# simonsobs/Pixell.jl

Measured on AMD Instinct MI355X. Metric: Mpix/s CAR bilinear reproject (Float64) + % HBM roofline, 1/2/4/8 MI355X, higher is better.
Workload: dtype f64

## Files before the change

pixell.jl_amd/csrc/pxl_kernels.hip:

```cpp
#include <hip/hip_runtime.h>

#include <algorithm>
#include <mutex>
#include <vector>
#include <cmath>
#include <cstdarg>
#include <cstdio>
#include <cstring>
#include <new>
#include <type_traits>

#include "pxl_device.h"

using namespace pxl;

static thread_local char g_err[512] = "";

static int fail(int code, const char* fmt, ...) {
    va_list ap;
    va_start(ap, fmt);
    vsnprintf(g_err, sizeof(g_err), fmt, ap);
    va_end(ap);
    return code;
}
// ... 387 lines not shown
                                    "this library can see is one it loaded itself (%s): a foreign communicator belongs to another instance", nc.where);
        int nranks = 0, me = -1;
        if (nc.CommCount((ncclComm_t)comm, &nranks) != ncclSuccess || nc.CommUserRank((ncclComm_t)comm, &me) != ncclSuccess)
            return fail(PXL_EINVAL, "sharded_step: not a usable RCCL communicator");
        for (int pass = 0; pass < 2; ++pass) {
            const pxl_halo_xfer* x = pass == 0 ? sends : recvs;
            for (int i = 0; i < (pass == 0 ? nsends : nrecvs); ++i) {
                if (x[i].peer < 0 || x[i].peer >= nranks) return fail(PXL_EINVAL, "sharded_step: peer %d outside the communicator (%d ranks)", x[i].peer, nranks);
                if (x[i].nrows < 1 || x[i].row0 < lo || x[i].row0 + x[i].nrows > hi) return fail(PXL_EINVAL, "sharded_step: transfer rows outside the plan's source window");
                if (pass == 0 && (x[i].row0 < own_row0 || x[i].row0 + x[i].nrows > own_row0 + own_nrows))
                    return fail(PXL_EINVAL, "sharded_step: a rank can only send rows it owns");
            }
        }
        if (!pl->comm_stream) {
            HIP_TRY(hipStreamCreateWithFlags(&pl->comm_stream, hipStreamNonBlocking));
            HIP_TRY(hipEventCreateWithFlags(&pl->ev_ready, hipEventDisableTiming));
            HIP_TRY(hipEventCreateWithFlags(&pl->ev_halo, hipEventDisableTiming));
        }
        HIP_TRY(hipEventRecord(pl->ev_ready, st));
        HIP_TRY(hipStreamWaitEvent(pl->comm_stream, pl->ev_ready, 0));
        const size_t esz = sizeof(T);
        const ncclDataType_t dt = std::is_same<T, float>::value ? ncclFloat32 : ncclFloat64;
        ncclResult_t r = nc.GroupStart();
        for (int i = 0; i < nsends && r == ncclSuccess; ++i)
            for (int64_t c = 0; c < pl->nc && r == ncclSuccess; ++c)
                r = nc.Send((const char*)src + ((c * pl->src_nrows + (sends[i].row0 - lo)) * pl->nx) * esz,
                            (size_t)(sends[i].nrows * pl->nx), dt, sends[i].peer, (ncclComm_t)comm, pl->comm_stream);
        for (int i = 0; i < nrecvs && r == ncclSuccess; ++i)
            for (int64_t c = 0; c < pl->nc && r == ncclSuccess; ++c)
                r = nc.Recv((char*)src + ((c * pl->src_nrows + (recvs[i].row0 - lo)) * pl->nx) * esz,
                            (size_t)(recvs[i].nrows * pl->nx), dt, recvs[i].peer, (ncclComm_t)comm, pl->comm_stream);
        const ncclResult_t rend = nc.GroupEnd();
        if (r == ncclSuccess) r = rend;
        if (r != ncclSuccess) return fail(PXL_EHIP, "sharded_step: RCCL send/recv failed: %s", nc.GetErrorString(r));
        HIP_TRY(hipEventRecord(pl->ev_halo, pl->comm_stream));
    }
    rc = pxl_reproject_build_tables(pl, stream);
    if (rc) return rc;
    int64_t i_lo = 0, i_hi = pl->dst_nrows;
    if (exchange) {
        if (pl->cov_have_lo != own_row0 || pl->cov_have_hi != own_row0 + own_nrows || pl->cov_hi < pl->cov_lo) {
            rc = pxl_reproject_plan_rows_covered(pl, own_row0, own_row0 + own_nrows, &pl->cov_lo, &pl->cov_hi);
            if (rc) return rc;
            pl->cov_have_lo = own_row0; pl->cov_have_hi = own_row0 + own_nrows;
        }
        i_lo = pl->cov_lo; i_hi = pl->cov_hi;
    }
    if (i_hi > i_lo) {
        rc = reproject_rows_impl<T>(pl, src, dst, i_lo, i_hi - i_lo, stream);
        if (rc) return rc;
    }
    if (exchange) {
        HIP_TRY(hipStreamWaitEvent(st, pl->ev_halo, 0));
        if (i_hi > i_lo) {
            if (i_lo > 0) { rc = reproject_rows_impl<T>(pl, src, dst, 0, i_lo, stream); if (rc) return rc; }
            if (i_hi < pl->dst_nrows) rc = reproject_rows_impl<T>(pl, src, dst, i_hi, pl->dst_nrows - i_hi, stream);
        } else {
            rc = reproject_rows_impl<T>(pl, src, dst, 0, pl->dst_nrows, stream);
        }
    }
    return rc;
}

static unsigned int* last_exact_word(int64_t total_tiles = -1, int64_t* total_out = nullptr) {
    DeviceState* d = device_state();
    if (!d) return nullptr;
    std::lock_guard<std::mutex> lock(g_dev_mu);
    if (!d->last_exact) {
        if (hipMalloc((void**)&d->last_exact, 64) != hipSuccess || hipMemset(d->last_exact, 0, 64) != hipSuccess) {
            (void)hipGetLastError(); d->last_exact = nullptr; return nullptr;
        }
    }
    if (total_tiles >= 0) d->generic_tiles = total_tiles;
    if (total_out) *total_out = d->generic_tiles;
    return d->last_exact;
}

static int generic_params(const char* who, const pxl_car_wcs* wcs_in, int proj_in, const int64_t* shape_in,
                          const pxl_car_wcs* wcs_out, int proj_out, const int64_t* shape_out, GenericParams* out) {
    if (!wcs_ok(wcs_in) || !wcs_ok(wcs_out)) return fail(PXL_EINVAL, "%s: invalid WCS", who);
    if (!shape_in || !shape_out) return fail(PXL_EINVAL, "%s: null shape", who);
    if (shape_in[0] < 1 || shape_in[1] < 1 || shape_out[0] < 1 || shape_out[1] < 1)
        return fail(PXL_EINVAL, "%s: shapes must be positive", who);
    if ((proj_in != PXL_PROJ_CAR && proj_in != PXL_PROJ_TAN) || (proj_out != PXL_PROJ_CAR && proj_out != PXL_PROJ_TAN))
        return fail(PXL_EINVAL, "%s: unknown projection code", who);
    GenericParams p;
    memset(&p, 0, sizeof(p));
    p.nx = shape_in[0]; p.ny = shape_in[1]; p.nc = 1;
    p.nxo = shape_out[0]; p.nyo = shape_out[1];
    p.proj_in = proj_in; p.proj_out = proj_out;
    p.periodic = (proj_in == PXL_PROJ_CAR) && car_periodic(wcs_in, p.nx);
    if (proj_out == PXL_PROJ_TAN) p.out_tan = tan_setup(*wcs_out); else p.out_car = car_affine(*wcs_out);
    if (proj_in == PXL_PROJ_TAN) p.in_tan = tan_setup(*wcs_in);
    else p.in_car = sky2pix_setup(*wcs_in, p.nx, p.ny, 1, PXL_FORM_DIV);
    *out = p;
    return PXL_OK;
}

struct LatticeWs { double2* lat; int32_t* flag; unsigned int* counter; size_t bytes; };
static LatticeWs lattice_layout(void* mem, int64_t ntiles) {
    const size_t lat_bytes = (size_t)ntiles * (PXL_TNX * PXL_TNY) * sizeof(double2), flag_bytes = ((size_t)ntiles * 4 + 15) & ~(size_t)15;
    const uintptr_t b = (uintptr_t)mem;
    return {(double2*)b, (int32_t*)(b + lat_bytes), (unsigned int*)(b + lat_bytes + flag_bytes), lat_bytes + flag_bytes + 16};
}
static hipError_t lattice_build(const GenericParams& p, int64_t gx, int64_t ntiles, const LatticeWs& ws, hipStream_t st) {
    hipError_t e = hipMemsetAsync(ws.counter, 0, 16, st);
    if (e == hipSuccess) hipLaunchKernelGGL(k_generic_lattice, dim3((unsigned)((ntiles + 3) / 4)), dim3(256), 0, st, p, gx, ntiles, ws.lat, ws.flag);
    return e;
}

static int check_sample(const char* who, const pxl_car_wcs* wcs_in, const int64_t shape_in[3], int64_t src_row0, int64_t src_nrows,
                        int64_t n, const double* sky, const void* out, bool no_data) {
    if (!wcs_ok(wcs_in) || !shape_in) return fail(PXL_EINVAL, "%s: invalid WCS/shape", who);
    if (shape_in[0] < 1 || shape_in[1] < 1 || shape_in[2] < 1) return fail(PXL_EINVAL, "%s: shapes must be positive", who);
    if (src_row0 < 0 || src_nrows < 0 || src_row0 + src_nrows > shape_in[1])
        return fail(PXL_EINVAL, "%s: source window outside the map", who);
    if (n < 0 || (n > 0 && (!sky || !out || no_data))) return fail(PXL_EINVAL, "%s: null buffer or negative n", who);
    if (((uintptr_t)sky & 15) != 0) return fail(PXL_EINVAL, "%s: 2xN buffer must be 16-byte aligned", who);
    return PXL_OK;
}

template <class T>
static int sample_impl(const pxl_car_wcs* wcs_in, const int64_t shape_in[3], const T* src, int64_t src_row0,
                       int64_t src_nrows, int64_t n, const double* sky, T* out, void* stream) {
    if (int rc = check_sample("sample", wcs_in, shape_in, src_row0, src_nrows, n, sky, out, !src && src_nrows > 0)) return rc;
    if (n == 0) return PXL_OK;
    Sky2Pix s = sky2pix_setup(*wcs_in, shape_in[0], shape_in[1], 1, PXL_FORM_RECIP);
    dim3 grid(stream_grid((n + PXL_SUNR - 1) / PXL_SUNR, 256));
    hipLaunchKernelGGL((k_sample_bilinear<T>), grid, dim3(256), 0, (hipStream_t)stream, s, src, shape_in[0], shape_in[1],
                       (int32_t)shape_in[2], src_row0, src_nrows, car_periodic(wcs_in, shape_in[0]), n, (const double2*)sky, out);
    return check_launch("k_sample_bilinear");
}

static int spline_shape_check(const char* what, const int64_t shape[3]) {
    if (!shape) return fail(PXL_EINVAL, "%s: null shape", what);
    if (shape[0] < 4 || shape[1] < 4) return fail(PXL_EINVAL, "%s: a cubic spline needs nx, ny >= 4 (got %lld x %lld)", what, (long long)shape[0], (long long)shape[1]);
    if (shape[2] < 1 || shape[2] > 65535) return fail(PXL_EINVAL, "%s: 1 to 65535 components", what);
    if (shape[0] > 400000000 || shape[1] > 400000000) return fail(PXL_EINVAL, "%s: axis too long (<= 4e8 pixels)", what);
    return PXL_OK;
}

template <class T>
static int build_pairs_impl(const int64_t shape_in[3], const T* src, int64_t src_nrows, T* pairs, void* stream) {
    if (pxl_sample_pairs_elems(shape_in, src_nrows) < 0) return PXL_EINVAL;
    if (!pairs || (!src && src_nrows > 0)) return fail(PXL_EINVAL, "sample_build_pairs: null buffer");
    if (((uintptr_t)pairs & 63) != 0) return fail(PXL_EINVAL, "sample_build_pairs: pair buffer must be 64-byte aligned");
    if (shape_in[0] > 0x7fffffffLL) return fail(PXL_EINVAL, "sample_build_pairs: more than 2^31 columns");
    if (shape_in[2] > 65535) return fail(PXL_EINVAL, "sample_build_pairs: more than 65535 components");
    const int64_t nx = shape_in[0], tiles = (src_nrows + 1 + PXL_POS_ROWS - 1) / PXL_POS_ROWS;
    if (tiles > 65535) return fail(PXL_EINVAL, "sample_build_pairs: more than %lld rows per call", 65535LL * PXL_POS_ROWS);
    const int64_t pitch = PairGroup<T>::groups(nx) * PairGroup<T>::E;
    const Fronts f = front_split(tiles, 16, 65535);
    dim3 grid((unsigned)((pitch + 255) / 256), (unsigned)(f.per * f.fronts), (unsigned)shape_in[2]);
    hipLaunchKernelGGL((k_build_rowpairs<T>), grid, dim3(256), 0, (hipStream_t)stream, src, nx, src_nrows, (typename Vec2T<T>::type*)pairs, f.fronts);
    return check_launch("k_build_rowpairs");
}

template <class T>
static int sample_pairs_impl(const pxl_car_wcs* wcs_in, const int64_t shape_in[3], const T* pairs, int64_t src_row0,
                             int64_t src_nrows, int64_t n, const double* sky, T* out, void* stream) {
    if (int rc = check_sample("sample_pairs", wcs_in, shape_in, src_row0, src_nrows, n, sky, out, !pairs)) return rc;
    if (((uintptr_t)pairs & 63) != 0) return fail(PXL_EINVAL, "sample_pairs: pair buffer must be 64-byte aligned");
    if (shape_in[0] > 0x7fffffffLL) return fail(PXL_EINVAL, "sample_pairs: more than 2^31 columns");
    if (n == 0) return PXL_OK;
    Sky2Pix s = sky2pix_setup(*wcs_in, shape_in[0], shape_in[1], 1, PXL_FORM_RECIP);
    dim3 grid(stream_grid((n + PairsUnroll<T>::value - 1) / PairsUnroll<T>::value, 256));
    hipLaunchKernelGGL((k_sample_pairs<T>), grid, dim3(256), 0, (hipStream_t)stream, s, (const typename Vec2T<T>::type*)pairs,
                       shape_in[0], shape_in[1], (int32_t)shape_in[2], src_row0, src_nrows, car_periodic(wcs_in, shape_in[0]), n,
                       (const double2*)sky, out);
    return check_launch("k_sample_pairs");
}

extern "C" {

int pxl_version(void) { return PXL_VERSION; }

size_t pxl_last_error(char* buf, size_t n) {
    size_t len = strlen(g_err);
    if (buf && n) {
        size_t m = len < n - 1 ? len : n - 1;
        memcpy(buf, g_err, m);
        buf[m] = 0;
    }
    return len;
}

int pxl_release_scratch(void) {
    DeviceState* d = device_state();
    if (!d) return fail(PXL_ENODEV, "release_scratch: no current device");
    std::lock_guard<std::mutex> lock(g_dev_mu);
    if (d->pool && hipMemPoolTrimTo(d->pool, 0) != hipSuccess) return fail(PXL_EHIP, "release_scratch: hipMemPoolTrimTo failed");
    return PXL_OK;
}

int pxl_mem_probe_pair(void* a, void* b, size_t window_bytes, int reps, float* us, void* stream) {
    if (!a || !b || !us) return fail(PXL_EINVAL, "mem_probe_pair: null argument");
    if (window_bytes < (64u << 20) || (window_bytes & 63) != 0 || (((uintptr_t)a | (uintptr_t)b) & 15) != 0)
        return fail(PXL_EINVAL, "mem_probe_pair: windows of at least 64 MiB, a multiple of 64 bytes, 16-byte aligned");
    if (reps < 1 || reps > 99) return fail(PXL_EINVAL, "mem_probe_pair: 1..99 repetitions");
    hipStream_t st = (hipStream_t)stream;
    hipEvent_t e0, e1;
    HIP_TRY(hipEventCreate(&e0));
    {
        hipError_t ec = hipEventCreate(&e1);
        if (ec != hipSuccess) { (void)hipEventDestroy(e0); return fail(PXL_EHIP, "hipEventCreate(&e1): %s", hipGetErrorString(ec)); }
    }
    std::vector<float> t(reps);
    int rc = PXL_OK;
    for (int r = -1; r < reps && rc == PXL_OK; ++r) {
        hipError_t e = hipEventRecord(e0, st);
        hipLaunchKernelGGL(k_spread_probe, dim3(8 * 256 * 2), dim3(256), 0, st, (char*)a, (char*)b, window_bytes / 4);
        if (e == hipSuccess) e = hipGetLastError();
        if (e == hipSuccess) e = hipEventRecord(e1, st);
        if (e == hipSuccess) e = hipEventSynchronize(e1);
        float ms = 0.f;
        if (e == hipSuccess) e = hipEventElapsedTime(&ms, e0, e1);
        if (e != hipSuccess) rc = fail(PXL_EHIP, "mem_probe_pair: %s", hipGetErrorString(e));
        else if (r >= 0) t[r] = ms * 1000.f;
    }
    (void)hipEventDestroy(e0);
    (void)hipEventDestroy(e1);
    if (rc) return rc;
    std::sort(t.begin(), t.end());
    *us = t[reps / 2];
    return PXL_OK;
}

#include "pxl_place.h"

int pxl_device_count(void) {
    int n = 0;
    hipError_t e = hipGetDeviceCount(&n);
    if (e != hipSuccess) return fail(PXL_ENODEV, "hipGetDeviceCount: %s", hipGetErrorString(e));
    return n;
}

int pxl_pix2sky_car_f64(const pxl_car_wcs* wcs, int64_t n, const double* pix, double* sky, int wrap_mode,
                        void* stream) {
    if (!wcs_ok(wcs)) return fail(PXL_EINVAL, "pix2sky: invalid WCS");
    if (n < 0 || (n > 0 && (!pix || !sky))) return fail(PXL_EINVAL, "pix2sky: null buffer or negative n");
    if (wrap_mode < PXL_WRAP_NONE || wrap_mode > PXL_WRAP_UNWIND) return fail(PXL_EINVAL, "pix2sky: bad wrap_mode %d", wrap_mode);
    if ((((uintptr_t)pix | (uintptr_t)sky) & 15) != 0) return fail(PXL_EINVAL, "pix2sky: 2xN buffers must be 16-byte aligned");
    if (n == 0) return PXL_OK;
    hipStream_t st = (hipStream_t)stream;
    CarAffine c = car_affine(*wcs);
    const int mode = wrap_mode == PXL_WRAP_REWIND ? 1 : (wrap_mode == PXL_WRAP_UNWIND ? 2 : 0);
    if (wrap_mode == PXL_WRAP_NONE) {
        hipLaunchKernelGGL((k_pix2sky_pairs<1>), dim3(stream_grid(n, 256)), dim3(256), 0, st, c, n, (const double2*)pix,
                           (double2*)sky, mode, (const int32_t*)nullptr);
        return check_launch("k_pix2sky_pairs");
    }
    const dim3 pgrid(stream_grid((n + 1) / 2, 256));
    if (wrap_mode != PXL_WRAP_UNWIND) {
        hipLaunchKernelGGL((k_pix2sky_pairs<2>), pgrid, dim3(256), 0, st, c, n, (const double2*)pix, (double2*)sky, mode,
                           (const int32_t*)nullptr);
        return check_launch("k_pix2sky_pairs");
    }
    const uintptr_t pa = (uintptr_t)pix, sa = (uintptr_t)sky, bytes = (uintptr_t)n * 16;
    if (pa != sa && pa < sa + bytes && sa < pa + bytes) return fail(PXL_EINVAL, "pix2sky: pix and sky may alias exactly or not at all");
    auto pre_rewind = [&](const int32_t* gate) {
        hipLaunchKernelGGL((k_pix2sky_pairs<2>), dim3(std::min(pgrid.x, 2048u)), dim3(256), 0, st, c, n, (const double2*)pix, (double2*)sky, 2, gate);
        return check_launch("k_pix2sky_pairs");
    };
    return unwind_ladder<true>(UwSrcPix2{c, (const double2*)pix, PXL_TWOPI_D, 0.0, 1.0 / PXL_TWOPI_D}, (double2*)sky, n, pa == sa, pre_rewind, st);
}

int pxl_rewind_f64(double* a, int64_t n, double period, double ref_angle, void* stream) {
    if (n < 0 || (n > 0 && !a)) return fail(PXL_EINVAL, "rewind: null buffer or negative n");
    if (!(period > 0.0) || !std::isfinite(period) || !std::isfinite(ref_angle)) return fail(PXL_EINVAL, "rewind: period must be positive and finite");
    if (n == 0) return PXL_OK;
    hipLaunchKernelGGL(k_rewind, dim3(stream_grid((n + 3) / 4, 256)), dim3(256), 0, (hipStream_t)stream, n, a, period, ref_angle, 0,
                       (const int32_t*)nullptr);
    return check_launch("k_rewind");
}

int pxl_unwind_f64(double* a, int64_t n, int nrow, double period, double ref_angle, void* stream) {
    if (n < 0 || (n > 0 && !a)) return fail(PXL_EINVAL, "unwind: null buffer or negative n");
    if (nrow != 1 && nrow != 2) return fail(PXL_EINVAL, "unwind: nrow must be 1 (vector) or 2 (2xN batch)");
    if (!(period > 0.0) || !std::isfinite(period) || !std::isfinite(ref_angle)) return fail(PXL_EINVAL, "unwind: period must be positive and finite");
    if (nrow == 2 && ((uintptr_t)a & 15) != 0) return fail(PXL_EINVAL, "unwind: 2xN buffer must be 16-byte aligned");
    if (n == 0) return PXL_OK;
    hipStream_t st = (hipStream_t)stream;
    const dim3 rgrid(stream_grid(((int64_t)nrow * n + 3) / 4, 256));
    auto pre_rewind = [&](const int32_t* gate) {
        hipLaunchKernelGGL(k_rewind, dim3(std::min(rgrid.x, 2048u)), dim3(256), 0, st, (int64_t)nrow * n, a, period, ref_angle, 1, gate);
        return check_launch("k_rewind");
    };
    if (nrow == 2) return unwind_ladder<false>(UwSrcAng2{(const double2*)a, period, ref_angle, 1.0 / period}, (double2*)a, n, true, pre_rewind, st);
    return unwind_ladder<false>(UwSrcAng1{(const double*)a, period, ref_angle, 1.0 / period}, a, n, true, pre_rewind, st);
}

int pxl_pix2sky_car_soa_f64(const pxl_car_wcs* wcs, int64_t n, const double* ipix, const double* jpix,
                            double* ra, double* dec, int safe, void* stream) {
    if (!wcs_ok(wcs)) return fail(PXL_EINVAL, "pix2sky_soa: invalid WCS");
    if (n < 0 || (n > 0 && (!ipix || !jpix || !ra || !dec))) return fail(PXL_EINVAL, "pix2sky_soa: null buffer or negative n");
    if (n == 0) return PXL_OK;
    const int vec = ((((uintptr_t)ipix | (uintptr_t)jpix | (uintptr_t)ra | (uintptr_t)dec) & 15) == 0) ? 1 : 0;
    hipLaunchKernelGGL(k_pix2sky_soa, dim3(stream_grid((n + 1) / 2, 256)), dim3(256), 0, (hipStream_t)stream,
                       car_affine(*wcs), n, ipix, jpix, ra, dec, safe ? 1 : 0, vec);
    return check_launch("k_pix2sky_soa");
}

int pxl_sky2pix_car_f64(const pxl_car_wcs* wcs, const int64_t shape[2], int64_t n, const double* sky,
                        double* pix, int safe, int form, void* stream) {
    if (!wcs_ok(wcs) || !shape) return fail(PXL_EINVAL, "sky2pix: invalid WCS/shape");
    if (n < 0 || (n > 0 && (!pix || !sky))) return fail(PXL_EINVAL, "sky2pix: null buffer or negative n");
    if (form < 0 || form > 2) return fail(PXL_EINVAL, "sky2pix: bad form %d", form);
// ... 668 lines not shown
```

pixell.jl_amd/csrc/pxl_sample.h:

```cpp
#pragma once

struct GenericParams {
    const double* src; double* dst;
    int64_t nx, ny, nxo, nyo;
    int32_t nc, periodic, proj_in, proj_out;
    CarAffine out_car; TanParams out_tan;
    Sky2Pix in_car; TanParams in_tan;
    unsigned int* exact_tiles;
    unsigned int* exact_tiles_last;
};
__device__ inline void generic_coords(const GenericParams& p, double i, double j, double* x, double* y, bool* visible) {
    double ra, dec;
    if (p.proj_out == PXL_PROJ_TAN) tan_pix2sky(p.out_tan, i, j, &ra, &dec);
    else { ra = p2s_ra(p.out_car, i); dec = p2s_dec(p.out_car, j); }
    *visible = true;
    if (p.proj_in == PXL_PROJ_TAN) {
        tan_sky2pix(p.in_tan, ra, dec, x, y);
        *visible = (p.in_tan.sd0 * sin(dec) + cos(dec) * cos(ra - p.in_tan.a0) * p.in_tan.cd0) > 0.0;
    } else { *x = s2p_x(p.in_car, ra); *y = s2p_y(p.in_car, dec); }
}
__device__ inline void generic_store(const GenericParams& p, int64_t t, double x, double y, bool visible) {
    const int64_t total = p.nxo * p.nyo;
    const bool fin = isfinite(x) && isfinite(y);
    int32_t i0, j0; double fx, fy;
// ... 192 lines not shown
#ifndef PXL_T3_G
#define PXL_T3_G 4
#endif

    constexpr int G = PXL_T3_G;
#pragma unroll
    for (int q0 = 0; q0 < NQ; q0 += G) {
        double fx[G], fy[G];
        int64_t off[G];
        bool ok = true;
#pragma unroll
        for (int g = 0; g < G; ++g) {
            const int r = ry + PXL_TROWS * (q0 + g);
            double x, y;
            coords(r, &x, &y);
            const double flx = floor(x), fly = floor(y);
            fx[g] = x - flx; fy[g] = y - fly;
            const int32_t i0 = (int32_t)flx, j0 = (int32_t)fly;
            ok = ok && (uint32_t)(i0 - 1) < nxm1 && (uint32_t)(j0 - 1) < nym1;
            off[g] = small ? (int64_t)((j0 - 1) * nx32 + (i0 - 1)) : (int64_t)(j0 - 1) * p.nx + (i0 - 1);
        }
        const bool inside = tj0 + ry + PXL_TROWS * (q0 + G - 1) < p.nyo;
        if (inside && __all(ok)) {
            for (int c = 0; c < p.nc; ++c) {
                const double* pl = p.src + (int64_t)c * p.nx * p.ny;
                Pair tp[G], bt[G];
#pragma unroll
                for (int g = 0; g < G; ++g) { tp[g] = *reinterpret_cast<const Pair*>(pl + off[g]); bt[g] = *reinterpret_cast<const Pair*>(pl + off[g] + p.nx); }
#pragma unroll
                for (int g = 0; g < G; ++g) {
                    const double top = (1 - fx[g]) * tp[g].a + fx[g] * tp[g].b;
                    const double bot = (1 - fx[g]) * bt[g].a + fx[g] * bt[g].b;
                    __builtin_nontemporal_store((1 - fy[g]) * top + fy[g] * bot, &p.dst[(int64_t)c * total + (tj0 + ry + PXL_TROWS * (q0 + g)) * p.nxo + i]);
                }
            }
        } else {
#pragma unroll
            for (int g = 0; g < G; ++g)
                if (tj0 + ry + PXL_TROWS * (q0 + g) < p.nyo) slow_rows |= 1u << (q0 + g);
        }
    }
#pragma unroll 1
    while (slow_rows) {
        const int q = __builtin_ctz(slow_rows);
        slow_rows &= slow_rows - 1;
        const int r = ry + PXL_TROWS * q;
        double x, y;
        double sx = 0.0, sy = 0.0;
#pragma unroll
        for (int b = 0; b < PXL_TNY; ++b) { const double wy = c_tile_weights.wy[r][b]; sx = __builtin_fma(wy, colx[b], sx); sy = __builtin_fma(wy, coly[b], sy); }
        x = sx; y = sy;
        generic_store(p, (tj0 + r) * p.nxo + i, x, y, true);
    }
}

#ifndef PXL_SUNR
#define PXL_SUNR 4
#endif
__device__ __noinline__ double2 sample_coords_slow(double a, double d, double ia0, double a0, double rda, double px, double cx,
                                                   double rpx, double id0, double d0, double rdd, double py, double cy, double rpy) {
    return make_double2(rewind(ia0 + (a - a0) * rda, px, cx, rpx), rewind(id0 + (d - d0) * rdd, py, cy, rpy));
}
__device__ inline void sample_coords(const Sky2Pix& s, double a, double d, double* x, double* y) {
    if (s.safe && s.form != PXL_FORM_DIV) {
        bool ok0, ok1;
        *x = rewind_try(s.c.ia0 + (a - s.c.a0) * s.rda, s.px, s.cx, s.rpx, &ok0);
        *y = rewind_try(s.c.id0 + (d - s.c.d0) * s.rdd, s.py, s.cy, s.rpy, &ok1);
        if (__builtin_expect(!(ok0 && ok1), 0)) {
            const double2 r = sample_coords_slow(a, d, s.c.ia0, s.c.a0, s.rda, s.px, s.cx, s.rpx, s.c.id0, s.c.d0, s.rdd, s.py, s.cy, s.rpy);
            *x = r.x; *y = r.y;
        }
        return;
    }
    *x = s2p_x(s, a); *y = s2p_y(s, d);
}
template <typename T>
__global__ __launch_bounds__(256) void k_sample_bilinear(Sky2Pix s, const T* __restrict__ src, int64_t nx,
                                                         int64_t ny, int32_t nc, int64_t row0, int64_t nrows,
                                                         int periodic, int64_t n, const double2* __restrict__ sky,
                                                         T* __restrict__ out) {
    const int64_t chunk = (int64_t)blockDim.x * PXL_SUNR;
    const int64_t plane = nx * nrows;
    for (int64_t k0 = (int64_t)blockIdx.x * chunk + threadIdx.x; k0 < n; k0 += (int64_t)gridDim.x * chunk) {
        double2 ad[PXL_SUNR];
#pragma unroll
        for (int u = 0; u < PXL_SUNR; ++u) {
            int64_t k = k0 + u * blockDim.x;
            ad[u] = (k < n) ? sky[k] : make_double2(0.0, 0.0);
        }
        int64_t o00[PXL_SUNR], o10[PXL_SUNR], o01[PXL_SUNR], o11[PXL_SUNR];
        double fx[PXL_SUNR], fy[PXL_SUNR];
        bool fin[PXL_SUNR];
#pragma unroll
        for (int u = 0; u < PXL_SUNR; ++u) {
            double x = s2p_x(s, ad[u].x), y = s2p_y(s, ad[u].y);
            fin[u] = isfinite(x) && isfinite(y);
            int32_t i0, j0;
            split_cell(x, &i0, &fx[u]);
            split_cell(y, &j0, &fy[u]);
            int64_t ia = i0, ib = (int64_t)i0 + 1;
            bool oka = true, okb = true;
            if (periodic) { ia = wrap_col(ia, nx); ib = wrap_col(ib, nx); }
            else { oka = (ia >= 1 && ia <= nx); okb = (ib >= 1 && ib <= nx); }
            int64_t ja = (int64_t)j0 - 1 - row0, jb = ja + 1;
            bool rowa = (j0 >= 1 && j0 <= ny && ja >= 0 && ja < nrows);
            bool rowb = ((int64_t)j0 + 1 >= 1 && (int64_t)j0 + 1 <= ny && jb >= 0 && jb < nrows);
            o00[u] = (rowa && oka) ? ja * nx + (ia - 1) : -1;
            o10[u] = (rowa && okb) ? ja * nx + (ib - 1) : -1;
            o01[u] = (rowb && oka) ? jb * nx + (ia - 1) : -1;
            o11[u] = (rowb && okb) ? jb * nx + (ib - 1) : -1;
        }
        for (int c = 0; c < nc; ++c) {
            const T* pl = src + (int64_t)c * plane;
            double m00[PXL_SUNR], m10[PXL_SUNR], m01[PXL_SUNR], m11[PXL_SUNR];
            struct __attribute__((packed, aligned(sizeof(T)))) TT { T a, b; };
            bool wide[PXL_SUNR];
#pragma unroll
            for (int u = 0; u < PXL_SUNR; ++u) {
                wide[u] = o00[u] >= 0 && o01[u] >= 0 && o10[u] == o00[u] + 1 && o11[u] == o01[u] + 1;
                const TT ra = *(wide[u] ? reinterpret_cast<const TT*>(pl + o00[u]) : reinterpret_cast<const TT*>(sky));
                const TT rb = *(wide[u] ? reinterpret_cast<const TT*>(pl + o01[u]) : reinterpret_cast<const TT*>(sky));
                m00[u] = (double)ra.a; m10[u] = (double)ra.b; m01[u] = (double)rb.a; m11[u] = (double)rb.b;
            }
#pragma unroll
            for (int u = 0; u < PXL_SUNR; ++u) {
                if (__builtin_expect(!wide[u], 0)) {
                    m00[u] = o00[u] >= 0 ? (double)pl[o00[u]] : 0.0;
                    m10[u] = o10[u] >= 0 ? (double)pl[o10[u]] : 0.0;
                    m01[u] = o01[u] >= 0 ? (double)pl[o01[u]] : 0.0;
                    m11[u] = o11[u] >= 0 ? (double)pl[o11[u]] : 0.0;
                }
            }
#pragma unroll
            for (int u = 0; u < PXL_SUNR; ++u) {
                int64_t k = k0 + u * blockDim.x;
                double top = (1 - fx[u]) * m00[u] + fx[u] * m10[u];
                double bot = (1 - fx[u]) * m01[u] + fx[u] * m11[u];
                double v = (1 - fy[u]) * top + fy[u] * bot;
                if (k < n) out[(int64_t)c * n + k] = (T)(fin[u] ? v : __builtin_nan(""));
            }
        }
    }
}

template <typename T> struct Vec2T;
template <> struct Vec2T<double> { typedef double2 type; };
template <> struct Vec2T<float>  { typedef float2 type; };

template <typename T> struct PairGroup {
    static constexpr int E = 64 / (2 * (int)sizeof(T));
    static constexpr int C = E - 1;
    __host__ __device__ static inline int64_t groups(int64_t nx) { return (nx + C - 1) / C; }
};
template <typename T>
__global__ __launch_bounds__(256) void k_build_rowpairs(const T* __restrict__ src, int64_t nx, int64_t nrows,
                                                        typename Vec2T<T>::type* __restrict__ pairs, int fronts) {
    typedef typename Vec2T<T>::type T2;
    constexpr int E = PairGroup<T>::E, C = PairGroup<T>::C;
    const int64_t pitch = PairGroup<T>::groups(nx) * E;
    const int64_t t = (int64_t)blockIdx.x * blockDim.x + threadIdx.x;
    if (t >= pitch) return;
    const int64_t g = t / E, e = t - g * E;
    int64_t i = g * C + e;
    if (i >= nx) i %= nx;
    const int64_t c = blockIdx.z;
    const T* pl = src + c * nx * nrows;
    T2* out = pairs + c * pitch * (nrows + 1);
    const int64_t per = (gridDim.y + fronts - 1) / fronts;
    const int64_t yy = fronts > 1 ? (int64_t)(blockIdx.y % fronts) * per + blockIdx.y / fronts : (int64_t)blockIdx.y;
    const int64_t p0 = yy * PXL_POS_ROWS;
    if (p0 > nrows) return;
    const int64_t p1 = (p0 + PXL_POS_ROWS <= nrows) ? p0 + PXL_POS_ROWS : nrows + 1;
    T above = (p0 >= 1) ? pl[(p0 - 1) * nx + i] : (T)0;
    for (int64_t p = p0; p < p1; ++p) {
        const T here = (p < nrows) ? pl[p * nx + i] : (T)0;
        T2 v; v.x = above; v.y = here;
        out[p * pitch + t] = v;
        above = here;
    }
}

template <typename T> struct PairsUnroll { static constexpr int value = PXL_SUNR; };
template <typename T>
__global__ __launch_bounds__(256) void k_sample_pairs(Sky2Pix s, const typename Vec2T<T>::type* __restrict__ pairs,
                                                      int64_t nx, int64_t ny, int32_t nc, int64_t row0, int64_t nrows,
                                                      int periodic, int64_t n, const double2* __restrict__ sky,
                                                      T* __restrict__ out) {
    typedef typename Vec2T<T>::type T2;
    constexpr int SUNR = PairsUnroll<T>::value;
    constexpr int E = PairGroup<T>::E, C = PairGroup<T>::C;
    const int64_t chunk = (int64_t)blockDim.x * SUNR;
    const int64_t pitch = PairGroup<T>::groups(nx) * E;
    const int64_t plane = pitch * (nrows + 1);
    for (int64_t k0 = (int64_t)blockIdx.x * chunk + threadIdx.x; k0 < n; k0 += (int64_t)gridDim.x * chunk) {
        double2 ad[SUNR];
#pragma unroll
        for (int u = 0; u < SUNR; ++u) {
            int64_t k = k0 + u * blockDim.x;
            ad[u] = (k < n) ? sky[k] : make_double2(0.0, 0.0);
        }
        int64_t oa[SUNR], ob[SUNR];
        double fx[SUNR], fy[SUNR];
        bool fin[SUNR];
#pragma unroll
        for (int u = 0; u < SUNR; ++u) {
            double x, y;
            sample_coords(s, ad[u].x, ad[u].y, &x, &y);
            fin[u] = isfinite(x) && isfinite(y);
            int32_t i0, j0;
            split_cell(x, &i0, &fx[u]);
            split_cell(y, &j0, &fy[u]);
            int64_t ia = i0, ib = (int64_t)i0 + 1;
            bool oka = true, okb = true;
            if (periodic) { ia = wrap_col(ia, nx); ib = wrap_col(ib, nx); }
            else { oka = (ia >= 1 && ia <= nx); okb = (ib >= 1 && ib <= nx); }
            const int64_t p = (int64_t)j0 - row0;
            const bool rows = (p >= 0 && p <= nrows);
            const uint32_t ca = (uint32_t)((oka ? ia : ib) - 1), ga = ca / (uint32_t)C;
            const int64_t ent = p * pitch + (int64_t)ga * E + (ca - ga * (uint32_t)C);
            oa[u] = (rows && oka) ? ent : -1;
            ob[u] = (rows && okb) ? (oka ? ent + 1 : ent) : -1;
        }
        for (int c = 0; c < nc; ++c) {
            const T2* pl = pairs + (int64_t)c * plane;
            T2 a[SUNR], b[SUNR];
#pragma unroll
            for (int u = 0; u < SUNR; ++u) {
                a[u] = pl[oa[u] >= 0 ? oa[u] : 0];
                b[u] = pl[ob[u] >= 0 ? ob[u] : 0];
            }
#pragma unroll
            for (int u = 0; u < SUNR; ++u) {
                if (oa[u] < 0) { a[u].x = (T)0; a[u].y = (T)0; }
                if (ob[u] < 0) { b[u].x = (T)0; b[u].y = (T)0; }
            }
#pragma unroll
            for (int u = 0; u < SUNR; ++u) {
                int64_t k = k0 + u * blockDim.x;
                double top = (1 - fx[u]) * (double)a[u].x + fx[u] * (double)b[u].x;
                double bot = (1 - fx[u]) * (double)a[u].y + fx[u] * (double)b[u].y;
                double v = (1 - fy[u]) * top + fy[u] * bot;
                if (k < n) out[(int64_t)c * n + k] = (T)(fin[u] ? v : __builtin_nan(""));
            }
        }
    }
}
```

Measured before the change: 394,200.

## Vectorize row-pair build with wide loads, wavefront shuffles and non-temporal stores

The row-pair staging kernel now has each wavefront load contiguous 16-byte vectors of source columns and redistribute them to the group-strided output lanes with __shfl. It also unrolls several rows per trip and writes the pair output with non-temporal stores. The goal is to replace scalar, partly duplicated gathers with fewer, wider loads and to cut cache pollution from the streaming writes. The cost is shuffle overhead, more complex indexing with a scalar fallback for unaligned widths, and added register pressure.

New measurement: 389,500. 1.2% lower.

```diff
diff --git a/pixell.jl_amd/csrc/pxl_kernels.hip b/pixell.jl_amd/csrc/pxl_kernels.hip
--- a/pixell.jl_amd/csrc/pxl_kernels.hip
+++ b/pixell.jl_amd/csrc/pxl_kernels.hip
@@ -563,7 +563,11 @@
     const int64_t pitch = PairGroup<T>::groups(nx) * PairGroup<T>::E;
     const Fronts f = front_split(tiles, 16, 65535);
     dim3 grid((unsigned)((pitch + 255) / 256), (unsigned)(f.per * f.fronts), (unsigned)shape_in[2]);
-    hipLaunchKernelGGL((k_build_rowpairs<T>), grid, dim3(256), 0, (hipStream_t)stream, src, nx, src_nrows, (typename Vec2T<T>::type*)pairs, f.fronts);
+    constexpr int V = 16 / (int)sizeof(T);
+    const bool vec = (nx % V) == 0 && ((uintptr_t)src & 15) == 0;
+    typename Vec2T<T>::type* out = (typename Vec2T<T>::type*)pairs;
+    if (vec) hipLaunchKernelGGL((k_build_rowpairs<T, V>), grid, dim3(256), 0, (hipStream_t)stream, src, nx, src_nrows, out, f.fronts);
+    else hipLaunchKernelGGL((k_build_rowpairs<T, 1>), grid, dim3(256), 0, (hipStream_t)stream, src, nx, src_nrows, out, f.fronts);
     return check_launch("k_build_rowpairs");
 }
 
diff --git a/pixell.jl_amd/csrc/pxl_sample.h b/pixell.jl_amd/csrc/pxl_sample.h
--- a/pixell.jl_amd/csrc/pxl_sample.h
+++ b/pixell.jl_amd/csrc/pxl_sample.h
@@ -368,31 +368,116 @@
     static constexpr int C = E - 1;
     __host__ __device__ static inline int64_t groups(int64_t nx) { return (nx + C - 1) / C; }
 };
-template <typename T>
+#ifndef PXL_PAIR_UNROLL
+#define PXL_PAIR_UNROLL 4
+#endif
+#ifndef PXL_PAIR_NT
+#define PXL_PAIR_NT 1
+#endif
+template <typename T, int V, bool WHOLE>
+__device__ __forceinline__ void pair_row_load(const T* __restrict__ row, int64_t c0, const int64_t (&col)[V], T (&r)[V]) {
+    if constexpr (WHOLE) {
+        typedef T TV __attribute__((ext_vector_type(V)));
+        const TV v = *reinterpret_cast<const TV*>(row + c0);
+#pragma unroll
+        for (int j = 0; j < V; ++j) r[j] = v[j];
+    } else {
+#pragma unroll
+        for (int j = 0; j < V; ++j) r[j] = row[col[j]];
+    }
+}
+template <typename T, int V>
+__device__ __forceinline__ T pair_row_exchange(const T (&r)[V], int from, int part) {
+    T here = __shfl(r[0], from);
+#pragma unroll
+    for (int j = 1; j < V; ++j) {
+        const T o = __shfl(r[j], from);
+        if (part == j) here = o;
+    }
+    return here;
+}
+template <typename T, int V, bool WHOLE, bool FULL>
+__device__ __forceinline__ void pair_rows_trip(const T* __restrict__ row, T __attribute__((ext_vector_type(2)))* __restrict__ o,
+                                               int64_t nx, int64_t nrows, int64_t pitch, int64_t p, int64_t p1, bool writes,
+                                               int64_t c0, const int64_t (&col)[V], int from, int part, T& above) {
+    typedef T TE __attribute__((ext_vector_type(2)));
+    constexpr int K = PXL_PAIR_UNROLL;
+    T r[K][V];
+#pragma unroll
+    for (int u = 0; u < K; ++u) {
+        if (FULL || p + u < nrows) pair_row_load<T, V, WHOLE>(row + u * nx, c0, col, r[u]);
+        else {
+#pragma unroll
+            for (int j = 0; j < V; ++j) r[u][j] = (T)0;
+        }
+    }
+#pragma unroll
+    for (int u = 0; u < K; ++u) {
+        if (FULL || p + u < p1) {
+            const T here = pair_row_exchange<T, V>(r[u], from, part);
+            TE v; v.x = above; v.y = here;
+            if (writes) {
+                if (PXL_PAIR_NT) __builtin_nontemporal_store(v, o + u * pitch);
+                else o[u * pitch] = v;
+            }
+            above = here;
+        }
+    }
+}
+template <typename T, int V, bool WHOLE>
+__device__ __forceinline__ void pair_rows_walk(const T* __restrict__ pl, typename Vec2T<T>::type* __restrict__ out, int64_t nx,
+                                               int64_t nrows, int64_t pitch, int64_t p0, int64_t p1, bool writes, int64_t c0,
+                                               const int64_t (&col)[V], int from, int part) {
+    typedef T TE __attribute__((ext_vector_type(2)));
+    constexpr int K = PXL_PAIR_UNROLL;
+    const T* row = pl + p0 * nx;
+    TE* o = reinterpret_cast<TE*>(out) + p0 * pitch;
+    T above = (T)0;
+    if (p0 >= 1) {
+        T r[V];
+        pair_row_load<T, V, WHOLE>(row - nx, c0, col, r);
+        above = pair_row_exchange<T, V>(r, from, part);
+    }
+    for (int64_t p = p0; p < p1; p += K, row += K * nx, o += K * pitch) {
+        if (p + K <= p1 && p + K <= nrows)
+            pair_rows_trip<T, V, WHOLE, true>(row, o, nx, nrows, pitch, p, p1, writes, c0, col, from, part, above);
+        else
+            pair_rows_trip<T, V, WHOLE, false>(row, o, nx, nrows, pitch, p, p1, writes, c0, col, from, part, above);
+    }
+}
+template <typename T, int V>
 __global__ __launch_bounds__(256) void k_build_rowpairs(const T* __restrict__ src, int64_t nx, int64_t nrows,
                                                         typename Vec2T<T>::type* __restrict__ pairs, int fronts) {
-    typedef typename Vec2T<T>::type T2;
     constexpr int E = PairGroup<T>::E, C = PairGroup<T>::C;
-    const int64_t pitch = PairGroup<T>::groups(nx) * E;
-    const int64_t t = (int64_t)blockIdx.x * blockDim.x + threadIdx.x;
-    if (t >= pitch) return;
-    const int64_t g = t / E, e = t - g * E;
-    int64_t i = g * C + e;
-    if (i >= nx) i %= nx;
+    constexpr int KW = 64 / E * C;
+    const int64_t ngroups = PairGroup<T>::groups(nx), pitch = ngroups * E;
+    const int lane = threadIdx.x & 63;
+    const int64_t w = (int64_t)blockIdx.x * (blockDim.x >> 6) + (threadIdx.x >> 6);
+    if (w * 64 >= pitch) return;
     const int64_t c = blockIdx.z;
     const T* pl = src + c * nx * nrows;
-    T2* out = pairs + c * pitch * (nrows + 1);
+    typename Vec2T<T>::type* out = pairs + c * pitch * (nrows + 1) + w * 64 + lane;
     const int64_t per = (gridDim.y + fronts - 1) / fronts;
     const int64_t yy = fronts > 1 ? (int64_t)(blockIdx.y % fronts) * per + blockIdx.y / fronts : (int64_t)blockIdx.y;
     const int64_t p0 = yy * PXL_POS_ROWS;
     if (p0 > nrows) return;
     const int64_t p1 = (p0 + PXL_POS_ROWS <= nrows) ? p0 + PXL_POS_ROWS : nrows + 1;
-    T above = (p0 >= 1) ? pl[(p0 - 1) * nx + i] : (T)0;
-    for (int64_t p = p0; p < p1; ++p) {
-        const T here = (p < nrows) ? pl[p * nx + i] : (T)0;
-        T2 v; v.x = above; v.y = here;
-        out[p * pitch + t] = v;
-        above = here;
+    const bool writes = w * 64 + lane < pitch;
+    const int64_t cw = w * KW;
+    const int64_t kmax = (ngroups * C - cw < KW) ? ngroups * C - cw : KW;
+    const int k0 = (lane * V <= kmax) ? lane * V : (int)(kmax / V) * V;
+    const int64_t c0 = cw + k0;
+    const int k = lane / E * C + lane % E;
+    const int from = k / V, part = k % V;
+    int64_t col[V];
+    if (V > 1 && __all(c0 + V - 1 < nx)) {
+#pragma unroll
+        for (int j = 0; j < V; ++j) col[j] = 0;
+        pair_rows_walk<T, V, true>(pl, out, nx, nrows, pitch, p0, p1, writes, c0, col, from, part);
+    } else {
+#pragma unroll
+        for (int j = 0; j < V; ++j) col[j] = (k0 + j > kmax) ? 0 : (c0 + j < nx) ? c0 + j : (c0 + j) % nx;
+        pair_rows_walk<T, V, false>(pl, out, nx, nrows, pitch, p0, p1, writes, c0, col, from, part);
     }
 }
 
```
